# sourmash-bio/sourmash

Hardware: AMD Instinct MI355X
Metric: Gbase/s sketched (k=31, scaled=1000) (higher is better)
Workload: dtype u64; 1 GPU; C2: sketch synthetic random DNA resident in HBM as ASCII, per GPU 1000 records of 10000000 bases (10000000000 bases, 10000001000 bytes with their separators), k=31 scaled=1000 seed=42; one step = k-mer kernel + radix sort + unique; records_per_gpu=1000, record_len=10000000, bases_per_gpu=10000000000, bytes_per_gpu=10000001000, ksize=31, scaled=1000, unique_hashes_rank0=9998668, unique_hashes_job=9998668, collectives=none (the exchange runs with --full)

## Files before the change

sourmash_amd/csrc/capi_ingest.cpp:

```cpp
#include <stdio.h>
#include <algorithm>
#include <atomic>
#include <chrono>
#include "capi_common.hpp"
#include "ingest.hpp"
#include "pargz.hpp"
#include "residues.hpp"
#include "sigload.hpp"
#include "uniform_sort_core.hpp"

using namespace smg;

namespace {

static size_t sketch_ws_raw_bytes(uint64_t cap) { return al256(cap * 8); }
static size_t sketch_ws_sort_bytes(uint64_t cap, bool counts) {
    return std::max(sort_unique_temp_bytes(cap), sort_unique_uniform_temp_bound(cap, counts));
}

struct SortCounters { std::atomic<uint64_t> bucket{0}, small{0}, fellback{0}; };
static SortCounters& sort_counters() { static SortCounters c; return c; }

static void uniform_sort_and_report(const uint64_t* d_keys, const unsigned long long* d_n, uint64_t n_max, uint64_t thr, uint64_t* d_out,
                                    uint64_t* d_counts, uint64_t* d_n_out, void* d_head, void* d_tmp, size_t tmp_bytes, hipStream_t st,
                                    uint64_t report[3]) {
    uint64_t* d_report = (uint64_t*)d_head;
    uint32_t* d_flag = (uint32_t*)((char*)d_head + 64);
    hip_check(sort_unique_uniform(d_keys, d_n, n_max, thr, d_out, d_counts, d_n_out, d_flag, d_tmp, tmp_bytes, st), "sort_unique_uniform");
    hip_check(sort_report_launch(d_n, d_n_out, d_flag, d_report, st), "sort_report");
    hip_check(hipMemcpyAsync(report, d_report, 24, hipMemcpyDeviceToHost, st), "D2H");
    hip_check(hipStreamSynchronize(st), "sync");
}
static void count_sort_call(uint64_t n_max, uint64_t thr, size_t tmp_bytes, bool counts, bool fellback) {
    if (fellback) ++sort_counters().fellback;
    else if (sort_unique_uniform_form(n_max, thr, tmp_bytes, counts) == US_SMALL) ++sort_counters().small;
    else ++sort_counters().bucket;
}
static int key_bits(uint64_t thr) {
    int bits = 64;
    if (thr != ~0ull) { bits = 1; while (bits < 64 && (thr >> bits)) ++bits; }
    return bits;
}

}

extern "C" {

uint64_t smgpu_signature_add_file(SourmashSignature* p, const char* path, uint64_t* n_records) {
    return landing<uint64_t>([&]() -> uint64_t {
        if (!path) throw err_internal("null path");
        std::vector<KmerMinHash*> mhs;
        for (auto& mh : SIG(p)->sketches) mhs.push_back(&mh);
        uint64_t recs = 0, bases = 0;
        sketch_file_into(mhs, path, &recs, &bases);
        if (n_records) *n_records = recs;
        return bases;
    });
}
SourmashSignature** smgpu_sketch_files(const char* const* paths, uintptr_t n, const SourmashComputeParameters* params,
                                       uint32_t n_threads, uint64_t* total_bases) {
    return landing<SourmashSignature**>([&]() -> SourmashSignature** {
        if (!paths && n) throw err_internal("null paths");
        if (!CP(params)->dna || CP(params)->protein || CP(params)->dayhoff || CP(params)->hp)
// ... 77 lines not shown
        if (!path) throw err_internal("null path");
        std::vector<KmerMinHash*> mhs{MH(p)};
        uint64_t recs = 0, bases = 0;
        sketch_file_into(mhs, path, &recs, &bases);
        if (n_records) *n_records = recs;
        return bases;
    });
}

uint64_t smgpu_sketch_workspace_bytes(uint64_t out_capacity) {
    return (uint64_t)sketch_ws_raw_bytes(out_capacity) + 256 + sketch_ws_sort_bytes(out_capacity, false) + 512;
}

void smgpu_sort_counters(uint64_t* out) {
    if (!out) return;
    out[0] = sort_counters().bucket.load();
    out[1] = sort_counters().small.load();
    out[2] = sort_counters().fellback.load();
}

uint64_t smgpu_sketch_dna_raw(const uint8_t* d_seq, uint64_t len, uint32_t ksize, uint64_t seed, uint64_t max_hash,
                              uint64_t* d_out, uint64_t cap, uint64_t* d_result, void* d_ws, uint64_t ws_bytes,
                              void* stream) {
    uint64_t ret = ~0ull;
    landing_void([&] {
        hipStream_t st = (hipStream_t)stream;
        if (ws_bytes < smgpu_sketch_workspace_bytes(cap)) throw err_internal("workspace too small (smgpu_sketch_workspace_bytes)");
        uint64_t* d_raw = (uint64_t*)d_ws;
        void* d_head = (char*)d_ws + sketch_ws_raw_bytes(cap);
        void* d_tmp = (char*)d_head + 256;
        const size_t tmp_bytes = (size_t)(ws_bytes - sketch_ws_raw_bytes(cap) - 256);
        const uint64_t thr = max_hash ? max_hash : ~0ull;
        check_dna_ksize(ksize);
        hip_check(hipMemsetAsync(d_result, 0, 16, st), "memset");
        hip_check(sketch_dna_launch(d_seq, len, ksize, seed, thr, d_raw, (unsigned long long*)d_result, cap, st), "sketch_dna");
        uint64_t report[3] = {0, 0, 0};
        uniform_sort_and_report(d_raw, (const unsigned long long*)d_result, cap, thr, d_out, nullptr, d_result + 1, d_head, d_tmp, tmp_bytes,
                                st, report);
        const uint64_t kept = report[0];
        if (kept > cap)
            throw err_internal("output capacity too small: " + std::to_string(kept) + " kept hashes > capacity " + std::to_string(cap));
        count_sort_call(cap, thr, tmp_bytes, false, report[2] != 0);
        if (report[2] == 0) { ret = report[1]; return; }
        hip_check(sort_unique(d_raw, kept, d_out, nullptr, d_result + 1, d_tmp, tmp_bytes, key_bits(thr), st), "sort_unique");
        unsigned long long nu = 0;
        hip_check(hipMemcpyAsync(&nu, d_result + 1, 8, hipMemcpyDeviceToHost, st), "D2H");
        hip_check(hipStreamSynchronize(st), "sync");
        ret = nu;
    });
    return ret;
}

uint64_t smgpu_sort_unique_uniform_workspace_bytes(uint64_t n_max, int32_t counts) {
    return 256 + (uint64_t)sketch_ws_sort_bytes(n_max, counts != 0) + 512;
}

uint64_t smgpu_sort_unique_uniform_raw(uint64_t* d_keys, const uint64_t* d_n, uint64_t n_max, uint64_t thr, uint64_t* d_out, uint64_t* d_counts,
                                       uint64_t* d_result, void* d_ws, uint64_t ws_bytes, void* stream) {
    uint64_t ret = ~0ull;
    landing_void([&] {
        hipStream_t st = (hipStream_t)stream;
        if (!d_keys || !d_n || !d_out || !d_result || !d_ws) throw err_internal("null pointer");
        if (ws_bytes < smgpu_sort_unique_uniform_workspace_bytes(n_max, d_counts != nullptr))
            throw err_internal("workspace too small (smgpu_sort_unique_uniform_workspace_bytes)");
        void* d_tmp = (char*)d_ws + 256;
        const size_t tmp_bytes = (size_t)(ws_bytes - 256);
        uint64_t report[3] = {0, 0, 0};
        uniform_sort_and_report(d_keys, (const unsigned long long*)d_n, n_max, thr, d_out, d_counts, d_result, d_ws, d_tmp, tmp_bytes, st, report);
        count_sort_call(n_max, thr, tmp_bytes, d_counts != nullptr, report[2] != 0);
        if (report[2] == 0) { ret = report[1]; return; }
        const uint64_t n = std::min(report[0], n_max);
        hip_check(sort_unique(d_keys, n, d_out, d_counts, d_result, d_tmp, tmp_bytes, 64, st), "sort_unique");
        unsigned long long nu = 0;
        hip_check(hipMemcpyAsync(&nu, d_result, 8, hipMemcpyDeviceToHost, st), "D2H");
        hip_check(hipStreamSynchronize(st), "sync");
        ret = nu;
    });
    return ret;
}

uint64_t smgpu_sort_unique_raw(uint64_t* d_keys, uint64_t n, uint64_t* d_out, uint64_t* d_n_out, void* d_ws, uint64_t ws_bytes, void* stream) {
    uint64_t ret = ~0ull;
    landing_void([&] {
        hipStream_t st = (hipStream_t)stream;
        if (ws_bytes < sort_unique_temp_bytes(n)) throw err_internal("workspace too small (smgpu_sketch_workspace_bytes)");
        hip_check(sort_unique(d_keys, n, d_out, nullptr, d_n_out, d_ws, (size_t)ws_bytes, 64, st), "sort_unique");
        unsigned long long nu = 0;
        hip_check(hipMemcpyAsync(&nu, d_n_out, 8, hipMemcpyDeviceToHost, st), "D2H");
        hip_check(hipStreamSynchronize(st), "sync");
        ret = nu;
    });
    return ret;
}

void smgpu_sketch_dna_kernel_raw(const uint8_t* d_seq, uint64_t len, uint32_t ksize, uint64_t seed, uint64_t max_hash,
                                 uint64_t* d_out, uint64_t cap, uint64_t* d_count, void* stream) {
    landing_void([&] {
        check_dna_ksize(ksize);
        hip_check(sketch_dna_launch(d_seq, len, ksize, seed, max_hash ? max_hash : ~0ull, d_out,
                                    (unsigned long long*)d_count, cap, (hipStream_t)stream), "sketch_dna");
// ... 94 lines not shown
```

sourmash_amd/csrc/device_api.hpp:

```cpp
#pragma once
#include <hip/hip_runtime.h>
#include <stdint.h>
#include <stddef.h>
#include "find_core.hpp"
#include "qindex_core.hpp"

namespace smg {

inline size_t al256(size_t x) { return (x + 255) / 256 * 256; }
inline unsigned grid_for(uint64_t n, unsigned per, unsigned cap) {
    const uint64_t b = (n + per - 1) / per;
    return (unsigned)(b < 1 ? 1 : (b > cap ? cap : b));
}

hipError_t sketch_dna_launch(const uint8_t* d_seq, uint64_t len, uint32_t k, uint64_t seed, uint64_t thr,
                             uint64_t* d_out, unsigned long long* d_count, uint64_t cap, hipStream_t stream);
hipError_t sketch_dna_launch_grid(const uint8_t* d_seq, uint64_t len, uint32_t k, uint64_t seed, uint64_t thr,
                                  uint64_t* d_out, unsigned long long* d_count, uint64_t cap, uint32_t grid, hipStream_t stream);
struct SketchMultiOut { uint64_t thr; uint64_t* out; unsigned long long* count; uint64_t cap; };
bool sketch_dna_multi_supported(const uint32_t* ks, int n);
hipError_t sketch_dna_multi_launch(const uint8_t* d_new, uint64_t n_new, const uint32_t* ks, int n, uint64_t seed, const SketchMultiOut* outs,
                                   hipStream_t stream);
hipError_t sketch_dna_words_launch(const uint8_t* d_seq, uint64_t len, uint32_t k, uint64_t seed, uint64_t thr, uint64_t* d_out,
                                   unsigned long long* d_count, uint64_t cap, bool dense, hipStream_t stream);
// ... 2 lines not shown
                              uint64_t n_kmers, hipStream_t stream);
hipError_t first_invalid_launch(const uint8_t* d_seq, uint64_t len, unsigned long long* d_first, hipStream_t stream);

hipError_t hll_dna_launch(const uint8_t* d_seq, uint64_t len, uint32_t k, uint32_t p, uint32_t* d_regs, hipStream_t stream);
hipError_t hll_hashes_launch(const uint64_t* d_hashes, uint64_t n, uint32_t p, uint32_t* d_regs, bool skip_zero, hipStream_t stream);
hipError_t hll_pack_launch(const uint32_t* d_regs, uint32_t n, uint8_t* d_out, hipStream_t stream);

struct NgTable { uint64_t size, magic, off; };
struct NgDev {
    const NgTable* tabs = nullptr;
    uint32_t n_tables = 0;
    uint32_t* words = nullptr;
    uint64_t n_words = 0;
    uint64_t t0_words = 0;
    unsigned long long* occ = nullptr;
};
hipError_t nodegraph_dna_launch(const uint8_t* d_seq, uint64_t len, uint32_t k, const NgDev& g, hipStream_t stream);
hipError_t nodegraph_hashes_launch(const uint64_t* d_hashes, uint64_t n, const NgDev& g, hipStream_t stream);
hipError_t nodegraph_matches_launch(const uint64_t* d_hashes, const uint64_t* d_offsets, uint64_t n_rows, const NgDev& g,
                                    uint64_t* d_out, hipStream_t stream);

hipError_t residues_launch(const uint8_t* d_seq, uint64_t len, uint32_t hash_function, uint8_t* d_aa, hipStream_t stream);
uint64_t translated_bytes(uint64_t len);
hipError_t translate_launch(const uint8_t* d_seq, uint64_t len, uint32_t hash_function, uint8_t* d_aa, hipStream_t stream);
hipError_t residue_windows_launch(const uint8_t* d_aa, uint64_t n, uint32_t k, uint64_t seed, uint64_t thr, uint64_t* d_out,
                                  unsigned long long* d_count, uint64_t cap, bool dense, hipStream_t stream);

size_t sort_unique_temp_bytes(uint64_t n);
struct TagSegment { uint64_t src, dst, n; };
hipError_t tag_gather_launch(const uint64_t* d_src, const TagSegment* d_segs, uint32_t n_segs, uint64_t* d_dst, int hbits, hipStream_t stream);
hipError_t sort_unique(uint64_t* d_keys, uint64_t n, uint64_t* d_out, uint64_t* d_counts, uint64_t* d_n_out,
                       void* d_temp, size_t temp_bytes, int bits, hipStream_t stream);

hipError_t sort_unique_uniform(const uint64_t* d_keys, const unsigned long long* d_n, uint64_t n_max, uint64_t thr, uint64_t* d_out,
                               uint64_t* d_counts, uint64_t* d_n_out, uint32_t* d_fellback, void* d_temp, size_t temp_bytes,
                               hipStream_t stream);
size_t sort_unique_uniform_temp_bytes(uint64_t n_max, uint64_t thr, bool counts);
size_t sort_unique_uniform_temp_bound(uint64_t n_max, bool counts);
uint32_t sort_unique_uniform_form(uint64_t n_max, uint64_t thr, size_t temp_bytes, bool counts);
hipError_t sort_report_launch(const unsigned long long* d_n, const uint64_t* d_n_out, const uint32_t* d_fellback, uint64_t* d_report,
                              hipStream_t stream);

size_t sort_pairs_temp_bytes(uint64_t n);
hipError_t sort_pairs(const uint64_t* d_keys_in, uint64_t* d_keys_out, const uint64_t* d_vals_in, uint64_t* d_vals_out, uint64_t n,
                      int bits, void* d_temp, size_t temp_bytes, hipStream_t stream);
size_t rle_pairs_temp_bytes(uint64_t n);
hipError_t rle_pairs(const uint64_t* d_a, const uint64_t* d_b, uint64_t n, uint64_t* d_out_a, uint64_t* d_out_b, uint64_t* d_counts,
                     uint64_t* d_n_out, void* d_temp, size_t temp_bytes, hipStream_t stream);

hipError_t records_pairs_launch(const uint8_t* d_seq, uint64_t len, uint32_t k, uint64_t seed, uint64_t thr, uint64_t* d_hash,
                                uint64_t* d_pos, unsigned long long* d_count, uint64_t cap, hipStream_t stream);
hipError_t records_check_starts_launch(const uint64_t* d_starts, uint64_t n_records, uint64_t len, unsigned long long* d_bad,
                                       hipStream_t stream);
size_t records_csr_temp_bytes(uint64_t n_pairs);
hipError_t records_csr_launch(uint64_t* d_pair_hash, uint64_t* d_pair_pos, uint64_t n_pairs, const uint64_t* d_starts, uint64_t n_records,
                              uint32_t k, uint64_t max_hash, uint64_t* d_hashes, uint64_t* d_abunds, uint64_t* d_offsets, uint64_t* d_n_out,
                              void* d_temp, size_t temp_bytes, hipStream_t stream);

hipError_t records_csr_ends_launch(uint64_t* d_pair_hash, uint64_t* d_pair_pos, uint64_t n_pairs, const uint64_t* d_starts, const uint64_t* d_ends,
                                   uint64_t n_records, uint32_t k, uint64_t max_hash, uint64_t* d_hashes, uint64_t* d_abunds, uint64_t* d_offsets,
                                   uint64_t* d_n_out, void* d_temp, size_t temp_bytes, hipStream_t stream);
hipError_t records_check_ends_launch(const uint64_t* d_starts, const uint64_t* d_ends, uint64_t n_records, unsigned long long* d_bad,
                                     hipStream_t stream);
hipError_t records_file_ends_launch(const uint64_t* d_starts, uint64_t n_records, uint64_t* d_ends, hipStream_t stream);

hipError_t residue_pairs_launch(const uint8_t* d_aa, uint64_t n_bound, const uint64_t* d_n, uint32_t k, uint64_t seed, uint64_t thr,
                                uint64_t* d_hash, uint64_t* d_pos, unsigned long long* d_count, uint64_t cap, hipStream_t stream);
uint64_t translated_records_bytes_bound(uint64_t len, uint64_t n_records);
size_t translate_records_temp_bytes(uint64_t n_records);
hipError_t translate_records_launch(const uint8_t* d_seq, uint64_t len, const uint64_t* d_starts, const uint64_t* d_ends, uint64_t n_records,
                                    uint32_t hash_function, uint64_t* d_block_starts, uint8_t* d_aa, void* d_temp, size_t temp_bytes,
                                    hipStream_t stream);

hipError_t find_dir_launch(const uint64_t* d_q, uint64_t n, uint32_t shift, uint64_t n_buckets, uint32_t* d_dir, hipStream_t stream);
// ... 153 lines not shown
```

sourmash_amd/csrc/uniform_sort.hip:

```cpp
#include <hip/hip_runtime.h>
#include "device_api.hpp"
#include "uniform_sort_core.hpp"

namespace smg {
namespace {

constexpr uint32_t NO_BASE = 0xffffffffu;

__device__ __forceinline__ uint64_t us_count(const unsigned long long* d_n, uint64_t n_max) {
    const uint64_t n = *d_n;
    return n < n_max ? n : n_max;
}

template <int T>
__device__ __forceinline__ void us_sort_lds(uint64_t* keys, uint32_t n) {
    const uint32_t P = us_pow2(n);
    for (uint32_t k = 2, j = 0; k <= P; us_next_step(k, j)) {
        for (uint32_t t = threadIdx.x; t < P / 2; t += T) {
            uint32_t a, b;
            us_pair(t, k, j, a, b);
            us_compare_exchange(keys, n, a, b);
        }
        __syncthreads();
    }
}

template <int T>
__device__ __forceinline__ uint32_t us_block_scan(uint32_t v, uint32_t* wsum, uint32_t& total) {
    const uint32_t lane = threadIdx.x & 63, wave = threadIdx.x >> 6;
    uint32_t x = v;
#pragma unroll
    for (uint32_t off = 1; off < 64; off <<= 1) {
        const uint32_t y = __shfl_up(x, off);
        if (lane >= off) x += y;
    }
    if (lane == 63) wsum[wave] = x;
    __syncthreads();
    uint32_t base = 0, all = 0;
#pragma unroll
    for (uint32_t w = 0; w < T / 64; ++w) {
        const uint32_t t = wsum[w];
        if (w < wave) base += t;
        all += t;
    }
    __syncthreads();
    total = all;
    return base + x - v;
}

template <int T, int E, int B, bool LEAF>
__device__ __forceinline__ void us_sort_keys(const uint64_t* src, uint32_t n, uint32_t bin_shift, uint64_t* s, uint32_t* bins,
                                             uint32_t* wsum) {
    constexpr int BPT = B / T;
    static_assert(B % T == 0, "bins per thread");
#pragma unroll
    for (int i = 0; i < BPT; ++i) bins[threadIdx.x + i * T] = 0;
    __syncthreads();
    uint64_t key[E];
    uint32_t at[E];
#pragma unroll
    for (int e = 0; e < E; ++e) {
        const uint32_t i = threadIdx.x + e * T;
        key[e] = 0;
        at[e] = 0;
        if (i < n) {
            key[e] = src[i];
            at[e] = atomicAdd(&bins[LEAF ? us_bin_leaf(bin_shift, key[e]) : us_bin_small(bin_shift, key[e])], 1u);
        }
    }
    __syncthreads();
    uint32_t mine[BPT], sum = 0, most = 0;
#pragma unroll
    for (int i = 0; i < BPT; ++i) {
        mine[i] = bins[threadIdx.x * BPT + i];
        sum += mine[i];
        most = mine[i] > most ? mine[i] : most;
    }
    uint32_t total;
    uint32_t start = us_block_scan<T>(sum, wsum, total);
    if (__syncthreads_or(most > US_BIN_LIMIT)) {
#pragma unroll
        for (int e = 0; e < E; ++e)
            if (threadIdx.x + e * T < n) s[threadIdx.x + e * T] = key[e];
        __syncthreads();
        us_sort_lds<T>(s, n);
        return;
    }
#pragma unroll
    for (int i = 0; i < BPT; ++i) {
        bins[threadIdx.x * BPT + i] = start;
        start += mine[i];
    }
    if (threadIdx.x == T - 1) bins[B] = start;
    __syncthreads();
#pragma unroll
    for (int e = 0; e < E; ++e) {
        if (threadIdx.x + e * T >= n) continue;
        at[e] += bins[LEAF ? us_bin_leaf(bin_shift, key[e]) : us_bin_small(bin_shift, key[e])];
        s[at[e]] = key[e];
// ... 18 lines not shown
template <int T, int E, typename CT>
__device__ __forceinline__ uint32_t us_unique_write(const uint64_t* keys, uint32_t n, uint32_t* scan, uint64_t* out, CT* counts) {
    const uint32_t lo = threadIdx.x * E;
    uint32_t heads = 0;
#pragma unroll
    for (int e = 0; e < E; ++e)
        if (lo + e < n && us_is_head(keys, lo + e)) ++heads;
    uint32_t total;
    const uint32_t first = us_block_scan<T>(heads, scan, total);
    uint32_t q = first;
#pragma unroll
    for (int e = 0; e < E; ++e) {
        const uint32_t i = lo + e;
        if (i < n && us_is_head(keys, i)) {
            out[q] = keys[i];
            if (counts) counts[q] = (CT)0 - (CT)i;
            ++q;
        }
    }
    if (counts) {
        __syncthreads();
        q = first;
#pragma unroll
        for (int e = 0; e < E; ++e) {
            const uint32_t i = lo + e;
            if (i >= n) break;
            if (us_is_head(keys, i)) ++q;
            if (us_is_tail(keys, n, i)) counts[q - 1] += (CT)(i + 1);
        }
    }
    return total;
}

__global__ __launch_bounds__(1024) void us_small_kernel(const uint64_t* __restrict__ keys, const unsigned long long* __restrict__ d_n,
                                                        uint64_t n_max, uint32_t small_shift, uint64_t* __restrict__ out,
                                                        uint64_t* __restrict__ counts, uint64_t* __restrict__ d_n_out,
                                                        uint32_t* __restrict__ d_fellback) {
    __shared__ uint64_t s[US_SMALL_MAX];
    __shared__ uint32_t bins[US_SMALL_BINS + 1];
    __shared__ uint32_t scan[1024 / 64];
    const uint32_t n = (uint32_t)us_count(d_n, n_max < US_SMALL_MAX ? n_max : US_SMALL_MAX);
    us_sort_keys<1024, US_SMALL_MAX / 1024, US_SMALL_BINS, false>(keys, n, small_shift, s, bins, scan);
    const uint32_t total = us_unique_write<1024, US_SMALL_MAX / 1024, uint64_t>(s, n, scan, out, counts);
    if (threadIdx.x == 0) {
        *d_n_out = total;
        *d_fellback = 0;
    }
}

template <bool SECOND>
__global__ __launch_bounds__(256) void us_scatter_kernel(const UsPlan p, const uint64_t* __restrict__ src,
                                                         const unsigned long long* __restrict__ d_n, uint64_t n_max,
                                                         const uint32_t* __restrict__ src_cursor, uint32_t tiles_per_region,
                                                         uint32_t* __restrict__ cursor, uint64_t* __restrict__ dst, uint64_t dst_cap,
                                                         uint32_t* __restrict__ d_fellback) {
    __shared__ uint32_t hist[US_FANOUT];
    __shared__ uint32_t base[US_FANOUT];
    uint64_t region = 0, begin, n;
    if (!SECOND) {
        n = us_count(d_n, n_max);
        begin = (uint64_t)blockIdx.x * US_TILE;
    } else {
        __shared__ uint32_t quit;
        if (threadIdx.x == 0) quit = *d_fellback;
        __syncthreads();
        if (quit) return;
        region = blockIdx.x / tiles_per_region;
        const uint64_t held = src_cursor[region];
        n = held < p.region_cap ? held : p.region_cap;
        begin = (uint64_t)(blockIdx.x % tiles_per_region) * US_TILE;
        src += region * p.region_cap;
        cursor += region * US_FANOUT;
        dst += region * US_FANOUT * dst_cap;
    }
    if (begin >= n) return;
    hist[threadIdx.x] = 0;
    __syncthreads();
    constexpr int E = US_TILE / 256;
    uint64_t key[E];
    uint32_t digit[E], rank[E];
    bool stray = false;
#pragma unroll
    for (int e = 0; e < E; ++e) {
        const uint64_t i = begin + (uint64_t)e * 256 + threadIdx.x;
        digit[e] = US_FANOUT;
        rank[e] = 0;
        key[e] = 0;
        if (i < n) {
            key[e] = src[i];
            digit[e] = SECOND ? us_digit_second(p, region, key[e]) : us_digit_first(p, key[e]);
            if (digit[e] < US_FANOUT) rank[e] = atomicAdd(&hist[digit[e]], 1u);
            else stray = true;
        }
    }
    if (stray) atomicOr(d_fellback, 1u);
    __syncthreads();
    {
        const uint32_t c = hist[threadIdx.x];
        uint32_t b = NO_BASE;
        if (c) {
            const uint32_t at = atomicAdd(&cursor[threadIdx.x], c);
            if (us_reserve_ok(at, c, dst_cap)) b = at;
            else atomicOr(d_fellback, 1u);
        }
        base[threadIdx.x] = b;
    }
    __syncthreads();
#pragma unroll
    for (int e = 0; e < E; ++e) {
        if (digit[e] >= US_FANOUT) continue;
        const uint32_t b = base[digit[e]];
        if (b != NO_BASE) dst[(uint64_t)digit[e] * dst_cap + b + rank[e]] = key[e];
    }
}

__global__ __launch_bounds__(256) void us_leaf_kernel(uint32_t shift, const uint32_t* __restrict__ cursor, uint64_t* __restrict__ leaves,
                                                      uint32_t* __restrict__ leaf_counts, uint32_t* __restrict__ leaf_distinct,
                                                      const uint32_t* __restrict__ d_fellback) {
    __shared__ uint64_t s[US_LEAF_CAP];
    __shared__ uint32_t bins[US_LEAF_BINS + 1];
    __shared__ uint32_t scan[256 / 64];
    if (*d_fellback) return;
    const uint64_t leaf = blockIdx.x;
    const uint32_t held = cursor[leaf];
    const uint32_t n = held < US_LEAF_CAP ? held : US_LEAF_CAP;
    uint64_t* mine = leaves + leaf * US_LEAF_CAP;
    us_sort_keys<256, US_LEAF_CAP / 256, US_LEAF_BINS, true>(mine, n, shift, s, bins, scan);
    const uint32_t total = us_unique_write<256, US_LEAF_CAP / 256, uint32_t>(s, n, scan, mine,
                                                                            leaf_counts ? leaf_counts + leaf * US_LEAF_CAP : nullptr);
    if (threadIdx.x == 0) leaf_distinct[leaf] = total;
}

__global__ __launch_bounds__(1024) void us_scan_kernel(const uint32_t* __restrict__ leaf_distinct, uint32_t n_leaves,
                                                       uint32_t* __restrict__ offsets, uint64_t* __restrict__ d_n_out,
                                                       const uint32_t* __restrict__ d_fellback) {
    __shared__ uint32_t wsum[1024 / 64];
    if (*d_fellback) return;
    uint32_t carry = 0;
    for (uint32_t base = 0; base < n_leaves; base += 4096) {
        const uint32_t l = base + threadIdx.x * 4;
        uint32_t v[4], sum = 0, total;
#pragma unroll
        for (int i = 0; i < 4; ++i) {
            v[i] = l + i < n_leaves ? leaf_distinct[l + i] : 0;
            sum += v[i];
        }
        uint32_t at = carry + us_block_scan<1024>(sum, wsum, total);
#pragma unroll
        for (int i = 0; i < 4; ++i) {
            if (l + i < n_leaves) offsets[l + i] = at;
            at += v[i];
        }
        carry += total;
    }
    if (threadIdx.x == 0) {
        offsets[n_leaves] = carry;
        *d_n_out = carry;
    }
}

__global__ __launch_bounds__(256) void us_pack_kernel(const uint64_t* __restrict__ leaves, const uint32_t* __restrict__ leaf_counts,
                                                      const uint32_t* __restrict__ offsets, uint64_t* __restrict__ out,
                                                      uint64_t* __restrict__ counts, const uint32_t* __restrict__ d_fellback) {
    if (*d_fellback) return;
    const uint64_t leaf = blockIdx.x;
    const uint32_t at = offsets[leaf], n = offsets[leaf + 1] - at;
    for (uint32_t i = threadIdx.x; i < n; i += 256) {
        out[at + i] = leaves[leaf * US_LEAF_CAP + i];
        if (counts) counts[at + i] = leaf_counts[leaf * US_LEAF_CAP + i];
    }
}

__global__ void us_report_kernel(const unsigned long long* __restrict__ d_n, const uint64_t* __restrict__ d_n_out,
                                 const uint32_t* __restrict__ d_fellback, uint64_t* __restrict__ report) {
    report[0] = *d_n;
    report[1] = *d_n_out;
    report[2] = *d_fellback;
}

size_t up256(size_t x) { return (x + 255) / 256 * 256; }

struct UsLayout {
    size_t coarse_cursors, leaf_cursors, cursor_bytes, distinct, offsets, coarse, leaves, counts, total;
};
UsLayout us_layout(const UsPlan& p, bool counts) {
    UsLayout y{};
    const size_t n_leaf_cursors = p.form == US_TWO_PASS ? (size_t)p.regions * US_FANOUT : US_FANOUT;
    y.coarse_cursors = 0;
    y.leaf_cursors = up256(US_FANOUT * 4);
    y.cursor_bytes = y.leaf_cursors + up256(n_leaf_cursors * 4);
    y.distinct = y.cursor_bytes;
    y.offsets = y.distinct + up256(n_leaf_cursors * 4);
    y.coarse = y.offsets + up256((n_leaf_cursors + 1) * 4);
    y.leaves = y.coarse + up256((size_t)p.regions * p.region_cap * 8);
    y.counts = y.leaves + up256((size_t)p.leaves * US_LEAF_CAP * 8);
    y.total = y.counts + (counts ? up256((size_t)p.leaves * US_LEAF_CAP * 4) : 0);
    return y;
}

}

size_t sort_unique_uniform_temp_bytes(uint64_t n_max, uint64_t thr, bool counts) {
    const UsPlan p = us_plan(n_max, thr);
    if (p.form == US_SMALL || p.form == US_DECLINE) return 256;
    return us_layout(p, counts).total;
}

size_t sort_unique_uniform_temp_bound(uint64_t n_max, bool counts) {
    if (n_max <= US_SMALL_MAX) return 256;
    return up256((size_t)n_max * 8 * 5 + (counts ? (size_t)n_max * 4 * 3 : 0) + ((size_t)8 << 20));
}

uint32_t sort_unique_uniform_form(uint64_t n_max, uint64_t thr, size_t temp_bytes, bool counts) {
    const UsPlan p = us_plan(n_max, thr);
    if (p.form == US_SMALL || p.form == US_DECLINE) return p.form;
    return temp_bytes < us_layout(p, counts).total ? (uint32_t)US_DECLINE : p.form;
}

hipError_t sort_unique_uniform(const uint64_t* d_keys, const unsigned long long* d_n, uint64_t n_max, uint64_t thr, uint64_t* d_out,
                               uint64_t* d_counts, uint64_t* d_n_out, uint32_t* d_fellback, void* d_temp, size_t temp_bytes,
                               hipStream_t stream) {
    const UsPlan p = us_plan(n_max, thr);
    const uint32_t form = sort_unique_uniform_form(n_max, thr, temp_bytes, d_counts != nullptr);
    if (form == US_SMALL) {
        hipLaunchKernelGGL(us_small_kernel, dim3(1), dim3(1024), 0, stream, d_keys, d_n, n_max, us_small_shift(thr), d_out, d_counts, d_n_out,
                           d_fellback);
        return hipGetLastError();
    }
    if (form == US_DECLINE) return hipMemsetD32Async((hipDeviceptr_t)d_fellback, 1, 1, stream);
    const UsLayout y = us_layout(p, d_counts != nullptr);
    char* base = (char*)d_temp;
    uint32_t* coarse_cursors = (uint32_t*)(base + y.coarse_cursors);
    uint32_t* leaf_cursors = (uint32_t*)(base + y.leaf_cursors);
    uint32_t* distinct = (uint32_t*)(base + y.distinct);
    uint32_t* offsets = (uint32_t*)(base + y.offsets);
    uint64_t* coarse = (uint64_t*)(base + y.coarse);
    uint64_t* leaves = (uint64_t*)(base + y.leaves);
    uint32_t* leaf_counts = d_counts ? (uint32_t*)(base + y.counts) : nullptr;
    hipError_t e = hipMemsetAsync(d_fellback, 0, 4, stream);
    if (e != hipSuccess) return e;
    e = hipMemsetAsync(base, 0, y.cursor_bytes, stream);
    if (e != hipSuccess) return e;
    const uint32_t tiles = (uint32_t)((n_max + US_TILE - 1) / US_TILE);
    if (form == US_ONE_PASS) {
        hipLaunchKernelGGL(us_scatter_kernel<false>, dim3(tiles), dim3(256), 0, stream, p, d_keys, d_n, n_max, (const uint32_t*)nullptr, 1u,
                           leaf_cursors, leaves, (uint64_t)US_LEAF_CAP, d_fellback);
    } else {
        hipLaunchKernelGGL(us_scatter_kernel<false>, dim3(tiles), dim3(256), 0, stream, p, d_keys, d_n, n_max, (const uint32_t*)nullptr, 1u,
                           coarse_cursors, coarse, p.region_cap, d_fellback);
        const uint32_t tpr = (uint32_t)((p.region_cap + US_TILE - 1) / US_TILE);
        hipLaunchKernelGGL(us_scatter_kernel<true>, dim3((uint32_t)p.regions * tpr), dim3(256), 0, stream, p, (const uint64_t*)coarse, d_n,
                           n_max, (const uint32_t*)coarse_cursors, tpr, leaf_cursors, leaves, (uint64_t)US_LEAF_CAP, d_fellback);
    }
    const uint32_t L = (uint32_t)p.leaves;
    hipLaunchKernelGGL(us_leaf_kernel, dim3(L), dim3(256), 0, stream, p.shift, (const uint32_t*)leaf_cursors, leaves, leaf_counts, distinct,
                       (const uint32_t*)d_fellback);
    hipLaunchKernelGGL(us_scan_kernel, dim3(1), dim3(1024), 0, stream, (const uint32_t*)distinct, L, offsets, d_n_out,
                       (const uint32_t*)d_fellback);
    hipLaunchKernelGGL(us_pack_kernel, dim3(L), dim3(256), 0, stream, (const uint64_t*)leaves, (const uint32_t*)leaf_counts,
                       (const uint32_t*)offsets, d_out, d_counts, (const uint32_t*)d_fellback);
    return hipGetLastError();
}

hipError_t sort_report_launch(const unsigned long long* d_n, const uint64_t* d_n_out, const uint32_t* d_fellback, uint64_t* d_report,
                              hipStream_t stream) {
    hipLaunchKernelGGL(us_report_kernel, dim3(1), dim3(1), 0, stream, d_n, d_n_out, d_fellback, d_report);
    return hipGetLastError();
}

}
```

sourmash_amd/csrc/uniform_sort_core.hpp:

```cpp
#pragma once
#include <stdint.h>

#if defined(__HIPCC__)
#include <hip/hip_runtime.h>
#endif

#ifndef SMG_HD
#if defined(__HIPCC__)
#define SMG_HD __host__ __device__ __forceinline__
#else
#define SMG_HD inline
#endif
#endif

namespace smg {

constexpr uint32_t US_SMALL_MAX = 16384;
constexpr uint32_t US_LEAF_CAP = 1024;
constexpr uint32_t US_FANOUT = 256;
constexpr uint32_t US_TILE = 4096;
constexpr uint64_t US_MAX_LEAVES = (uint64_t)US_FANOUT * US_FANOUT;

enum UsForm : uint32_t { US_DECLINE = 0, US_SMALL = 1, US_ONE_PASS = 2, US_TWO_PASS = 3 };

// ... 24 lines not shown
    UsPlan p{US_DECLINE, 0, 0, 0, 0, thr};
    if (n_max <= US_SMALL_MAX) { p.form = US_SMALL; return p; }
    if (n_max > 0xffffffffull) return p;
    int shift = 63;
    for (; shift >= 0; --shift) {
        const uint64_t L = us_leaves(thr, (uint32_t)shift);
        if (L > US_MAX_LEAVES) return p;
        if (us_load_fits((n_max + L - 1) / L, US_LEAF_CAP)) break;
    }
    if (shift < 0) return p;
    p.shift = (uint32_t)shift;
    p.leaves = us_leaves(thr, p.shift);
    if (p.leaves <= US_FANOUT) { p.form = US_ONE_PASS; return p; }
    p.form = US_TWO_PASS;
    p.regions = ((p.leaves - 1) >> 8) + 1;
    const uint64_t load = ((n_max + p.leaves - 1) / p.leaves) * US_FANOUT;
    p.region_cap = load + 8 * us_isqrt_up(load);
    return p;
}

SMG_HD uint64_t us_leaf_of(const UsPlan& p, uint64_t key) { return key >> p.shift; }
SMG_HD uint32_t us_digit_first(const UsPlan& p, uint64_t key) {
    if (key > p.thr) return US_FANOUT;
    const uint64_t leaf = us_leaf_of(p, key);
    return (uint32_t)(p.form == US_TWO_PASS ? leaf >> 8 : leaf);
}
SMG_HD uint32_t us_digit_second(const UsPlan& p, uint64_t region, uint64_t key) {
    if (key > p.thr) return US_FANOUT;
    const uint64_t leaf = us_leaf_of(p, key);
    return (leaf >> 8) == region ? (uint32_t)(leaf & 0xff) : US_FANOUT;
}
SMG_HD bool us_reserve_ok(uint64_t base, uint64_t count, uint64_t cap) { return base <= cap && count <= cap - base; }

constexpr uint32_t US_LEAF_BINS = 1024;
constexpr uint32_t US_SMALL_BINS = 4096;
constexpr uint32_t US_BIN_LIMIT = 32;
SMG_HD uint32_t us_bin_leaf(uint32_t shift, uint64_t key) { return (uint32_t)(key >> (shift > 10 ? shift - 10 : 0)) & (US_LEAF_BINS - 1); }
SMG_HD uint32_t us_small_shift(uint64_t thr) {
    uint32_t s = 0;
    while (s < 63 && (thr >> s) >= US_SMALL_BINS) ++s;
    return s;
}
SMG_HD uint32_t us_bin_small(uint32_t small_shift, uint64_t key) {
    const uint64_t b = key >> small_shift;
    return b < US_SMALL_BINS ? (uint32_t)b : US_SMALL_BINS - 1;
}
SMG_HD bool us_before(uint64_t other, uint32_t other_at, uint64_t key, uint32_t at) { return other < key || (other == key && other_at < at); }

SMG_HD uint32_t us_pow2(uint32_t n) {
    uint32_t p = 1;
    while (p < n) p <<= 1;
    return p;
}
SMG_HD void us_pair(uint32_t t, uint32_t k, uint32_t j, uint32_t& a, uint32_t& b) {
    const uint32_t off = t & ((j == 0 ? k >> 1 : j) - 1);
    a = 2 * (t - off) + off;
    b = j == 0 ? 2 * (t - off) + k - 1 - off : a + j;
}
SMG_HD void us_compare_exchange(uint64_t* keys, uint32_t n, uint32_t a, uint32_t b) {
    if (b >= n) return;
    const uint64_t x = keys[a], y = keys[b];
    if (x > y) { keys[a] = y; keys[b] = x; }
}
SMG_HD void us_next_step(uint32_t& k, uint32_t& j) {
    if (j == 0) j = k >> 2; else j >>= 1;
    if (j == 0) k <<= 1;
// ... 7 lines not shown
```

Before: 384.9 Gbase/s.

## Restructure uniform sort scatter into persistent staged kernel and fold report writes

```diff
diff --git a/sourmash_amd/csrc/capi_ingest.cpp b/sourmash_amd/csrc/capi_ingest.cpp
--- a/sourmash_amd/csrc/capi_ingest.cpp
+++ b/sourmash_amd/csrc/capi_ingest.cpp
@@ -24,11 +24,8 @@
 static void uniform_sort_and_report(const uint64_t* d_keys, const unsigned long long* d_n, uint64_t n_max, uint64_t thr, uint64_t* d_out,
                                     uint64_t* d_counts, uint64_t* d_n_out, void* d_head, void* d_tmp, size_t tmp_bytes, hipStream_t st,
                                     uint64_t report[3]) {
-    uint64_t* d_report = (uint64_t*)d_head;
-    uint32_t* d_flag = (uint32_t*)((char*)d_head + 64);
-    hip_check(sort_unique_uniform(d_keys, d_n, n_max, thr, d_out, d_counts, d_n_out, d_flag, d_tmp, tmp_bytes, st), "sort_unique_uniform");
-    hip_check(sort_report_launch(d_n, d_n_out, d_flag, d_report, st), "sort_report");
-    hip_check(hipMemcpyAsync(report, d_report, 24, hipMemcpyDeviceToHost, st), "D2H");
+    hip_check(sort_unique_uniform(d_keys, d_n, n_max, thr, d_out, d_counts, d_n_out, d_head, d_tmp, tmp_bytes, st), "sort_unique_uniform");
+    hip_check(hipMemcpyAsync(report, (const char*)d_head + US_HEAD_REPORT, 24, hipMemcpyDeviceToHost, st), "D2H");
     hip_check(hipStreamSynchronize(st), "sync");
 }
 static void count_sort_call(uint64_t n_max, uint64_t thr, size_t tmp_bytes, bool counts, bool fellback) {
@@ -172,7 +169,7 @@
         const size_t tmp_bytes = (size_t)(ws_bytes - sketch_ws_raw_bytes(cap) - 256);
         const uint64_t thr = max_hash ? max_hash : ~0ull;
         check_dna_ksize(ksize);
-        hip_check(hipMemsetAsync(d_result, 0, 16, st), "memset");
+        hip_check(sort_unique_uniform_prepare(cap, thr, false, d_head, d_tmp, tmp_bytes, d_result, st), "sort_unique_uniform_prepare");
         hip_check(sketch_dna_launch(d_seq, len, ksize, seed, thr, d_raw, (unsigned long long*)d_result, cap, st), "sketch_dna");
         uint64_t report[3] = {0, 0, 0};
         uniform_sort_and_report(d_raw, (const unsigned long long*)d_result, cap, thr, d_out, nullptr, d_result + 1, d_head, d_tmp, tmp_bytes,
@@ -206,6 +203,7 @@
         void* d_tmp = (char*)d_ws + 256;
         const size_t tmp_bytes = (size_t)(ws_bytes - 256);
         uint64_t report[3] = {0, 0, 0};
+        hip_check(sort_unique_uniform_prepare(n_max, thr, d_counts != nullptr, d_ws, d_tmp, tmp_bytes, nullptr, st), "sort_unique_uniform_prepare");
         uniform_sort_and_report(d_keys, (const unsigned long long*)d_n, n_max, thr, d_out, d_counts, d_result, d_ws, d_tmp, tmp_bytes, st, report);
         count_sort_call(n_max, thr, tmp_bytes, d_counts != nullptr, report[2] != 0);
         if (report[2] == 0) { ret = report[1]; return; }
diff --git a/sourmash_amd/csrc/device_api.hpp b/sourmash_amd/csrc/device_api.hpp
--- a/sourmash_amd/csrc/device_api.hpp
+++ b/sourmash_amd/csrc/device_api.hpp
@@ -58,14 +58,15 @@
 hipError_t sort_unique(uint64_t* d_keys, uint64_t n, uint64_t* d_out, uint64_t* d_counts, uint64_t* d_n_out,
                        void* d_temp, size_t temp_bytes, int bits, hipStream_t stream);
 
+constexpr size_t US_HEAD_REPORT = 0;
+constexpr size_t US_HEAD_FLAG = 64;
+hipError_t sort_unique_uniform_prepare(uint64_t n_max, uint64_t thr, bool counts, void* d_head, void* d_temp, size_t temp_bytes,
+                                       uint64_t* d_result, hipStream_t stream);
 hipError_t sort_unique_uniform(const uint64_t* d_keys, const unsigned long long* d_n, uint64_t n_max, uint64_t thr, uint64_t* d_out,
-                               uint64_t* d_counts, uint64_t* d_n_out, uint32_t* d_fellback, void* d_temp, size_t temp_bytes,
-                               hipStream_t stream);
+                               uint64_t* d_counts, uint64_t* d_n_out, void* d_head, void* d_temp, size_t temp_bytes, hipStream_t stream);
 size_t sort_unique_uniform_temp_bytes(uint64_t n_max, uint64_t thr, bool counts);
 size_t sort_unique_uniform_temp_bound(uint64_t n_max, bool counts);
 uint32_t sort_unique_uniform_form(uint64_t n_max, uint64_t thr, size_t temp_bytes, bool counts);
-hipError_t sort_report_launch(const unsigned long long* d_n, const uint64_t* d_n_out, const uint32_t* d_fellback, uint64_t* d_report,
-                              hipStream_t stream);
 
 size_t sort_pairs_temp_bytes(uint64_t n);
 hipError_t sort_pairs(const uint64_t* d_keys_in, uint64_t* d_keys_out, const uint64_t* d_vals_in, uint64_t* d_vals_out, uint64_t n,
diff --git a/sourmash_amd/csrc/uniform_sort.hip b/sourmash_amd/csrc/uniform_sort.hip
--- a/sourmash_amd/csrc/uniform_sort.hip
+++ b/sourmash_amd/csrc/uniform_sort.hip
@@ -1,4 +1,5 @@
 #include <hip/hip_runtime.h>
+#include <stdlib.h>
 #include "device_api.hpp"
 #include "uniform_sort_core.hpp"
 
@@ -48,9 +49,18 @@
     return base + x - v;
 }
 
-template <int T, int E, int B, bool LEAF>
-__device__ __forceinline__ void us_sort_keys(const uint64_t* src, uint32_t n, uint32_t bin_shift, uint64_t* s, uint32_t* bins,
-                                             uint32_t* wsum) {
+template <int T, int E>
+__device__ __forceinline__ void us_load_keys(const uint64_t* src, uint32_t n, uint64_t (&key)[E]) {
+#pragma unroll
+    for (int e = 0; e < E; ++e) {
+        const uint32_t i = threadIdx.x + e * T;
+        key[e] = i < n ? src[i] : 0;
+    }
+}
+
+template <int T, int E, int B, bool LEAF, bool LOAD>
+__device__ __forceinline__ void us_sort_keys(const uint64_t (&held)[E], const uint64_t* src, uint32_t n, uint32_t bin_shift, uint64_t* s,
+                                             uint32_t* bins, uint32_t* wsum) {
     constexpr int BPT = B / T;
     static_assert(B % T == 0, "bins per thread");
 #pragma unroll
@@ -61,10 +71,10 @@
 #pragma unroll
     for (int e = 0; e < E; ++e) {
         const uint32_t i = threadIdx.x + e * T;
-        key[e] = 0;
         at[e] = 0;
+        key[e] = LOAD ? 0 : held[e];
         if (i < n) {
-            key[e] = src[i];
+            if (LOAD) key[e] = src[i];
             at[e] = atomicAdd(&bins[LEAF ? us_bin_leaf(bin_shift, key[e]) : us_bin_small(bin_shift, key[e])], 1u);
         }
     }
@@ -149,91 +159,188 @@
     return total;
 }
 
+__device__ __forceinline__ void us_write_report(void* d_head, uint64_t count, uint64_t distinct, uint32_t fellback) {
+    uint64_t* report = (uint64_t*)((char*)d_head + US_HEAD_REPORT);
+    report[0] = count;
+    report[1] = distinct;
+    report[2] = fellback;
+}
+__device__ __forceinline__ uint32_t* us_head_flag(void* d_head) { return (uint32_t*)((char*)d_head + US_HEAD_FLAG); }
+
+__global__ __launch_bounds__(256) void us_zero_kernel(uint32_t* __restrict__ words, uint32_t n_words, void* __restrict__ d_head,
+                                                      uint32_t* __restrict__ d_result32) {
+    const uint32_t i = blockIdx.x * 256 + threadIdx.x;
+    if (i < n_words) words[i] = 0;
+    if (i == 0) *us_head_flag(d_head) = 0;
+    if (d_result32 && i >= 1 && i < 5) d_result32[i - 1] = 0;
+}
+
+__global__ void us_decline_kernel(const unsigned long long* __restrict__ d_n, void* __restrict__ d_head) {
+    *us_head_flag(d_head) = 1;
+    us_write_report(d_head, *d_n, 0, 1);
+}
+
 __global__ __launch_bounds__(1024) void us_small_kernel(const uint64_t* __restrict__ keys, const unsigned long long* __restrict__ d_n,
                                                         uint64_t n_max, uint32_t small_shift, uint64_t* __restrict__ out,
                                                         uint64_t* __restrict__ counts, uint64_t* __restrict__ d_n_out,
-                                                        uint32_t* __restrict__ d_fellback) {
+                                                        void* __restrict__ d_head) {
     __shared__ uint64_t s[US_SMALL_MAX];
     __shared__ uint32_t bins[US_SMALL_BINS + 1];
     __shared__ uint32_t scan[1024 / 64];
     const uint32_t n = (uint32_t)us_count(d_n, n_max < US_SMALL_MAX ? n_max : US_SMALL_MAX);
-    us_sort_keys<1024, US_SMALL_MAX / 1024, US_SMALL_BINS, false>(keys, n, small_shift, s, bins, scan);
+    const uint64_t none[US_SMALL_MAX / 1024] = {};
+    us_sort_keys<1024, US_SMALL_MAX / 1024, US_SMALL_BINS, false, true>(none, keys, n, small_shift, s, bins, scan);
     const uint32_t total = us_unique_write<1024, US_SMALL_MAX / 1024, uint64_t>(s, n, scan, out, counts);
     if (threadIdx.x == 0) {
         *d_n_out = total;
-        *d_fellback = 0;
-    }
-}
+        *us_head_flag(d_head) = 0;
+        us_write_report(d_head, *d_n, total, 0);
+    }
+}
+
+struct UsTileAt {
+    const uint64_t* src;
+    uint32_t n;
+    uint32_t region;
+};
 
 template <bool SECOND>
-__global__ __launch_bounds__(256) void us_scatter_kernel(const UsPlan p, const uint64_t* __restrict__ src,
+__global__ __launch_bounds__(256, 4) void us_scatter_kernel(const UsPlan p, const uint64_t* __restrict__ src,
                                                          const unsigned long long* __restrict__ d_n, uint64_t n_max,
-                                                         const uint32_t* __restrict__ src_cursor, uint32_t tiles_per_region,
-                                                         uint32_t* __restrict__ cursor, uint64_t* __restrict__ dst, uint64_t dst_cap,
-                                                         uint32_t* __restrict__ d_fellback) {
-    __shared__ uint32_t hist[US_FANOUT];
-    __shared__ uint32_t base[US_FANOUT];
-    uint64_t region = 0, begin, n;
-    if (!SECOND) {
-        n = us_count(d_n, n_max);
-        begin = (uint64_t)blockIdx.x * US_TILE;
-    } else {
-        __shared__ uint32_t quit;
+                                                         const uint32_t* __restrict__ src_cursor, uint32_t* __restrict__ cursor,
+                                                         uint64_t* __restrict__ dst, uint64_t dst_cap, uint32_t* __restrict__ d_fellback) {
+    constexpr int E = US_TILE / 256;
+    __shared__ uint64_t stage[US_TILE];
+    __shared__ uint32_t hist[US_FANOUT * US_HIST_STRIDE];
+    __shared__ uint32_t lstart[US_FANOUT + 1];
+    __shared__ uint32_t tile_start[SECOND ? US_FANOUT + 1 : 1];
+    __shared__ uint32_t wsum[256 / 64];
+    __shared__ uint32_t quit;
+    const uint64_t n_first = us_count(d_n, n_max);
+    uint64_t n_tiles = us_tiles(n_first);
+    if (SECOND) {
+        if (blockIdx.x >= n_tiles + p.regions) return;
+        uint32_t mine = 0;
+        if (threadIdx.x < p.regions) {
+            const uint64_t held = src_cursor[threadIdx.x];
+            mine = (uint32_t)us_tiles(held < p.region_cap ? held : p.region_cap);
+        }
         if (threadIdx.x == 0) quit = *d_fellback;
+        uint32_t all;
+        const uint32_t at = us_block_scan<256>(mine, wsum, all);
+        tile_start[threadIdx.x] = at;
+        if (threadIdx.x == 255) tile_start[US_FANOUT] = all;
         __syncthreads();
         if (quit) return;
-        region = blockIdx.x / tiles_per_region;
-        const uint64_t held = src_cursor[region];
-        n = held < p.region_cap ? held : p.region_cap;
-        begin = (uint64_t)(blockIdx.x % tiles_per_region) * US_TILE;
-        src += region * p.region_cap;
-        cursor += region * US_FANOUT;
-        dst += region * US_FANOUT * dst_cap;
-    }
-    if (begin >= n) return;
-    hist[threadIdx.x] = 0;
-    __syncthreads();
-    constexpr int E = US_TILE / 256;
-    uint64_t key[E];
-    uint32_t digit[E], rank[E];
-    bool stray = false;
-#pragma unroll
-    for (int e = 0; e < E; ++e) {
-        const uint64_t i = begin + (uint64_t)e * 256 + threadIdx.x;
-        digit[e] = US_FANOUT;
-        rank[e] = 0;
-        key[e] = 0;
-        if (i < n) {
-            key[e] = src[i];
-            digit[e] = SECOND ? us_digit_second(p, region, key[e]) : us_digit_first(p, key[e]);
-            if (digit[e] < US_FANOUT) rank[e] = atomicAdd(&hist[digit[e]], 1u);
-            else stray = true;
-        }
-    }
-    if (stray) atomicOr(d_fellback, 1u);
-    __syncthreads();
-    {
-        const uint32_t c = hist[threadIdx.x];
-        uint32_t b = NO_BASE;
-        if (c) {
-            const uint32_t at = atomicAdd(&cursor[threadIdx.x], c);
-            if (us_reserve_ok(at, c, dst_cap)) b = at;
-            else atomicOr(d_fellback, 1u);
-        }
-        base[threadIdx.x] = b;
-    }
-    __syncthreads();
-#pragma unroll
-    for (int e = 0; e < E; ++e) {
-        if (digit[e] >= US_FANOUT) continue;
-        const uint32_t b = base[digit[e]];
-        if (b != NO_BASE) dst[(uint64_t)digit[e] * dst_cap + b + rank[e]] = key[e];
+        n_tiles = all;
+    }
+    if (blockIdx.x >= n_tiles) return;
+
+    auto tile_at = [&](uint64_t t) {
+        UsTileAt a;
+        if constexpr (!SECOND) {
+            const uint64_t begin = t * US_TILE, left = n_first - begin;
+            a.src = src + begin;
+            a.n = (uint32_t)(left < US_TILE ? left : US_TILE);
+            a.region = 0;
+        } else {
+            a.region = us_tile_region(tile_start, (uint32_t)t);
+            const uint64_t held = src_cursor[a.region];
+            const uint64_t n = held < p.region_cap ? held : p.region_cap;
+            const uint64_t begin = (t - tile_start[a.region]) * US_TILE, left = n - begin;
+            a.src = src + a.region * p.region_cap + begin;
+            a.n = (uint32_t)(left < US_TILE ? left : US_TILE);
+        }
+        return a;
+    };
+    auto load = [&](const UsTileAt& a, uint64_t (&key)[E]) {
+#pragma unroll
+        for (int e = 0; e < E; ++e) {
+            const uint32_t i = (uint32_t)e * 256 + threadIdx.x;
+            key[e] = i < a.n ? a.src[i] : 0;
+        }
+    };
+
+    const uint32_t sub = us_sub(threadIdx.x);
+#pragma unroll
+    for (uint32_t s = 0; s < US_SUBS; ++s) hist[us_hist_at(threadIdx.x, s)] = 0;
+    uint64_t key[E], next_key[E];
+    UsTileAt cur = tile_at(blockIdx.x), next = cur;
+    load(cur, key);
+    __syncthreads();
+    for (uint64_t t = blockIdx.x; t < n_tiles; t += gridDim.x) {
+        const bool more = t + gridDim.x < n_tiles;
+        if (threadIdx.x == 0) quit = __hip_atomic_load(d_fellback, __ATOMIC_RELAXED, __HIP_MEMORY_SCOPE_AGENT);
+        if (more) {
+            next = tile_at(t + gridDim.x);
+            load(next, next_key);
+        }
+        uint32_t* my_cursor = cursor + (SECOND ? (uint64_t)cur.region * US_FANOUT : 0);
+        uint64_t* my_dst = dst + (SECOND ? (uint64_t)cur.region * US_FANOUT * dst_cap : 0);
+        uint32_t where[E];
+        bool stray = false;
+#pragma unroll
+        for (int e = 0; e < E; ++e) {
+            where[e] = US_FANOUT << 12;
+            if ((uint32_t)e * 256 + threadIdx.x < cur.n) {
+                const uint32_t digit = SECOND ? us_digit_second(p, cur.region, key[e]) : us_digit_first(p, key[e]);
+                if (digit < US_FANOUT) where[e] = digit << 12 | atomicAdd(&hist[us_hist_at(digit, sub)], 1u);
+                else stray = true;
+            }
+        }
+        if (stray) atomicOr(d_fellback, 1u);
+        __syncthreads();
+        if (quit) return;
+        uint32_t c = 0;
+#pragma unroll
+        for (uint32_t s = 0; s < US_SUBS; ++s) {
+            const uint32_t v = hist[us_hist_at(threadIdx.x, s)];
+            hist[us_hist_at(threadIdx.x, s)] = c;
+            c += v;
+        }
+        {
+            uint32_t b = NO_BASE;
+            if (c) {
+                const uint32_t at = atomicAdd(&my_cursor[threadIdx.x], c);
+                if (us_reserve_ok(at, c, dst_cap)) b = at;
+                else atomicOr(d_fellback, 1u);
+            }
+            hist[us_hist_at(threadIdx.x, US_SUBS)] = b;
+        }
+        uint32_t placed;
+        const uint32_t first = us_block_scan<256>(c, wsum, placed);
+        lstart[threadIdx.x] = first;
+        __syncthreads();
+#pragma unroll
+        for (int e = 0; e < E; ++e) {
+            const uint32_t digit = where[e] >> 12;
+            if (digit < US_FANOUT) stage[lstart[digit] + hist[us_hist_at(digit, sub)] + (where[e] & 0xfffu)] = key[e];
+        }
+        __syncthreads();
+#pragma unroll
+        for (uint32_t s = 0; s < US_SUBS; ++s) hist[us_hist_at(threadIdx.x, s)] = 0;
+#pragma unroll
+        for (int e = 0; e < E; ++e) {
+            const uint32_t j = (uint32_t)e * 256 + threadIdx.x;
+            if (j >= placed) continue;
+            const uint64_t k = stage[j];
+            const uint32_t digit = SECOND ? us_digit_second(p, cur.region, k) : us_digit_first(p, k);
+            const uint32_t b = hist[us_hist_at(digit, US_SUBS)];
+            if (b != NO_BASE) my_dst[(uint64_t)digit * dst_cap + b + (j - lstart[digit])] = k;
+        }
+        if (more) {
+#pragma unroll
+            for (int e = 0; e < E; ++e) key[e] = next_key[e];
+            cur = next;
+        }
+        __syncthreads();
     }
 }
 
 __global__ __launch_bounds__(256) void us_leaf_kernel(uint32_t shift, const uint32_t* __restrict__ cursor, uint64_t* __restrict__ leaves,
                                                       uint32_t* __restrict__ leaf_counts, uint32_t* __restrict__ leaf_distinct,
                                                       const uint32_t* __restrict__ d_fellback) {
+    constexpr int E = US_LEAF_CAP / 256;
     __shared__ uint64_t s[US_LEAF_CAP];
     __shared__ uint32_t bins[US_LEAF_BINS + 1];
     __shared__ uint32_t scan[256 / 64];
@@ -242,29 +349,33 @@
     const uint32_t held = cursor[leaf];
     const uint32_t n = held < US_LEAF_CAP ? held : US_LEAF_CAP;
     uint64_t* mine = leaves + leaf * US_LEAF_CAP;
-    us_sort_keys<256, US_LEAF_CAP / 256, US_LEAF_BINS, true>(mine, n, shift, s, bins, scan);
-    const uint32_t total = us_unique_write<256, US_LEAF_CAP / 256, uint32_t>(s, n, scan, mine,
-                                                                            leaf_counts ? leaf_counts + leaf * US_LEAF_CAP : nullptr);
+    uint64_t key[E];
+    us_load_keys<256, E>(mine, n, key);
+    us_sort_keys<256, E, US_LEAF_BINS, true, false>(key, nullptr, n, shift, s, bins, scan);
+    const uint32_t total = us_unique_write<256, E, uint32_t>(s, n, scan, mine, leaf_counts ? leaf_counts + leaf * US_LEAF_CAP : nullptr);
     if (threadIdx.x == 0) leaf_distinct[leaf] = total;
 }
 
 __global__ __launch_bounds__(1024) void us_scan_kernel(const uint32_t* __restrict__ leaf_distinct, uint32_t n_leaves,
-                                                       uint32_t* __restrict__ offsets, uint64_t* __restrict__ d_n_out,
-                                                       const uint32_t* __restrict__ d_fellback) {
+                                                       uint32_t* __restrict__ offsets, const unsigned long long* __restrict__ d_n,
+                                                       uint64_t* __restrict__ d_n_out, void* __restrict__ d_head) {
     __shared__ uint32_t wsum[1024 / 64];
-    if (*d_fellback) return;
+    if (*us_head_flag(d_head)) {
+        if (threadIdx.x == 0) us_write_report(d_head, *d_n, 0, 1);
+        return;
+    }
     uint32_t carry = 0;
-    for (uint32_t base = 0; base < n_leaves; base += 4096) {
-        const uint32_t l = base + threadIdx.x * 4;
-        uint32_t v[4], sum = 0, total;
-#pragma unroll
-        for (int i = 0; i < 4; ++i) {
+    for (uint32_t base = 0; base < n_leaves; base += 1024 * US_SCAN_PER_LANE) {
+        const uint32_t l = base + threadIdx.x * US_SCAN_PER_LANE;
+        uint32_t v[US_SCAN_PER_LANE], sum = 0, total;
+#pragma unroll
+        for (uint32_t i = 0; i < US_SCAN_PER_LANE; ++i) {
             v[i] = l + i < n_leaves ? leaf_distinct[l + i] : 0;
             sum += v[i];
         }
         uint32_t at = carry + us_block_scan<1024>(sum, wsum, total);
 #pragma unroll
-        for (int i = 0; i < 4; ++i) {
+        for (uint32_t i = 0; i < US_SCAN_PER_LANE; ++i) {
             if (l + i < n_leaves) offsets[l + i] = at;
             at += v[i];
         }
@@ -273,6 +384,7 @@
     if (threadIdx.x == 0) {
         offsets[n_leaves] = carry;
         *d_n_out = carry;
+        us_write_report(d_head, *d_n, carry, 0);
     }
 }
 
@@ -286,13 +398,6 @@
         out[at + i] = leaves[leaf * US_LEAF_CAP + i];
         if (counts) counts[at + i] = leaf_counts[leaf * US_LEAF_CAP + i];
     }
-}
-
-__global__ void us_report_kernel(const unsigned long long* __restrict__ d_n, const uint64_t* __restrict__ d_n_out,
-                                 const uint32_t* __restrict__ d_fellback, uint64_t* __restrict__ report) {
-    report[0] = *d_n;
-    report[1] = *d_n_out;
-    report[2] = *d_fellback;
 }
 
 size_t up256(size_t x) { return (x + 255) / 256 * 256; }
@@ -334,17 +439,61 @@
     return temp_bytes < us_layout(p, counts).total ? (uint32_t)US_DECLINE : p.form;
 }
 
+namespace {
+
+unsigned us_grid_cap() {
+    static const unsigned cap = [] {
+        const char* e = getenv("SMG_US_GRID");
+        const long v = e ? atol(e) : 0;
+        return v > 0 ? (unsigned)v : 0xffffffffu;
+    }();
+    return cap;
+}
+
+unsigned us_resident(const void* kernel) {
+    int per_cu = 0, dev = 0, cus = 0;
+    if (hipOccupancyMaxActiveBlocksPerMultiprocessor(&per_cu, kernel, 256, 0) != hipSuccess || hipGetDevice(&dev) != hipSuccess ||
+        hipDeviceGetAttribute(&cus, hipDeviceAttributeMultiprocessorCount, dev) != hipSuccess || per_cu < 1 || cus < 1) {
+        (void)hipGetLastError();
+        return 1024u;
+    }
+    return (unsigned)per_cu * (unsigned)cus;
+}
+unsigned us_grid(unsigned resident, uint64_t work) {
+    uint64_t g = resident < us_grid_cap() ? resident : us_grid_cap();
+    if (g > work) g = work;
+    return g ? (unsigned)g : 1u;
+}
+
+}
+
+hipError_t sort_unique_uniform_prepare(uint64_t n_max, uint64_t thr, bool counts, void* d_head, void* d_temp, size_t temp_bytes,
+                                       uint64_t* d_result, hipStream_t stream) {
+    const uint32_t form = sort_unique_uniform_form(n_max, thr, temp_bytes, counts);
+    uint32_t n_words = 0;
+    if (form == US_ONE_PASS || form == US_TWO_PASS) n_words = (uint32_t)(us_layout(us_plan(n_max, thr), counts).cursor_bytes / 4);
+    else if (!d_result) return hipSuccess;
+    const uint32_t blocks = n_words > 5 ? (n_words + 255) / 256 : 1;
+    hipLaunchKernelGGL(us_zero_kernel, dim3(blocks), dim3(256), 0, stream, (uint32_t*)d_temp, n_words, d_head, (uint32_t*)d_result);
+    return hipGetLastError();
+}
+
 hipError_t sort_unique_uniform(const uint64_t* d_keys, const unsigned long long* d_n, uint64_t n_max, uint64_t thr, uint64_t* d_out,
-                               uint64_t* d_counts, uint64_t* d_n_out, uint32_t* d_fellback, void* d_temp, size_t temp_bytes,
-                               hipStream_t stream) {
+                               uint64_t* d_counts, uint64_t* d_n_out, void* d_head, void* d_temp, size_t temp_bytes, hipStream_t stream) {
     const UsPlan p = us_plan(n_max, thr);
     const uint32_t form = sort_unique_uniform_form(n_max, thr, temp_bytes, d_counts != nullptr);
+    uint32_t* d_fellback = (uint32_t*)((char*)d_head + US_HEAD_FLAG);
     if (form == US_SMALL) {
         hipLaunchKernelGGL(us_small_kernel, dim3(1), dim3(1024), 0, stream, d_keys, d_n, n_max, us_small_shift(thr), d_out, d_counts, d_n_out,
-                           d_fellback);
+                           d_head);
         return hipGetLastError();
     }
-    if (form == US_DECLINE) return hipMemsetD32Async((hipDeviceptr_t)d_fellback, 1, 1, stream);
+    if (form == US_DECLINE) {
+        hipLaunchKernelGGL(us_decline_kernel, dim3(1), dim3(1), 0, stream, d_n, d_head);
+        return hipGetLastError();
+    }
+    static const unsigned resident_first = us_resident((const void*)us_scatter_kernel<false>);
+    static const unsigned resident_second = us_resident((const void*)us_scatter_kernel<true>);
     const UsLayout y = us_layout(p, d_counts != nullptr);
     char* base = (char*)d_temp;
     uint32_t* coarse_cursors = (uint32_t*)(base + y.coarse_cursors);
@@ -354,35 +503,24 @@
     uint64_t* coarse = (uint64_t*)(base + y.coarse);
     uint64_t* leaves = (uint64_t*)(base + y.leaves);
     uint32_t* leaf_counts = d_counts ? (uint32_t*)(base + y.counts) : nullptr;
-    hipError_t e = hipMemsetAsync(d_fellback, 0, 4, stream);
-    if (e != hipSuccess) return e;
-    e = hipMemsetAsync(base, 0, y.cursor_bytes, stream);
-    if (e != hipSuccess) return e;
-    const uint32_t tiles = (uint32_t)((n_max + US_TILE - 1) / US_TILE);
+    const uint64_t tiles = us_tiles(n_max);
     if (form == US_ONE_PASS) {
-        hipLaunchKernelGGL(us_scatter_kernel<false>, dim3(tiles), dim3(256), 0, stream, p, d_keys, d_n, n_max, (const uint32_t*)nullptr, 1u,
-                           leaf_cursors, leaves, (uint64_t)US_LEAF_CAP, d_fellback);
+        hipLaunchKernelGGL(us_scatter_kernel<false>, dim3(us_grid(resident_first, tiles)), dim3(256), 0, stream, p, d_keys, d_n, n_max,
+                           (const uint32_t*)nullptr, leaf_cursors, leaves, (uint64_t)US_LEAF_CAP, d_fellback);
     } else {
-        hipLaunchKernelGGL(us_scatter_kernel<false>, dim3(tiles), dim3(256), 0, stream, p, d_keys, d_n, n_max, (const uint32_t*)nullptr, 1u,
-                           coarse_cursors, coarse, p.region_cap, d_fellback);
-        const uint32_t tpr = (uint32_t)((p.region_cap + US_TILE - 1) / US_TILE);
-        hipLaunchKernelGGL(us_scatter_kernel<true>, dim3((uint32_t)p.regions * tpr), dim3(256), 0, stream, p, (const uint64_t*)coarse, d_n,
-                           n_max, (const uint32_t*)coarse_cursors, tpr, leaf_cursors, leaves, (uint64_t)US_LEAF_CAP, d_fellback);
+        hipLaunchKernelGGL(us_scatter_kernel<false>, dim3(us_grid(resident_first, tiles)), dim3(256), 0, stream, p, d_keys, d_n, n_max,
+                           (const uint32_t*)nullptr, coarse_cursors, coarse, p.region_cap, d_fellback);
+        hipLaunchKernelGGL(us_scatter_kernel<true>, dim3(us_grid(resident_second, tiles + p.regions)), dim3(256), 0, stream, p,
+                           (const uint64_t*)coarse, d_n, n_max, (const uint32_t*)coarse_cursors, leaf_cursors, leaves, (uint64_t)US_LEAF_CAP,
+                           d_fellback);
     }
     const uint32_t L = (uint32_t)p.leaves;
     hipLaunchKernelGGL(us_leaf_kernel, dim3(L), dim3(256), 0, stream, p.shift, (const uint32_t*)leaf_cursors, leaves, leaf_counts, distinct,
                        (const uint32_t*)d_fellback);
-    hipLaunchKernelGGL(us_scan_kernel, dim3(1), dim3(1024), 0, stream, (const uint32_t*)distinct, L, offsets, d_n_out,
-                       (const uint32_t*)d_fellback);
+    hipLaunchKernelGGL(us_scan_kernel, dim3(1), dim3(1024), 0, stream, (const uint32_t*)distinct, L, offsets, d_n, d_n_out, d_head);
     hipLaunchKernelGGL(us_pack_kernel, dim3(L), dim3(256), 0, stream, (const uint64_t*)leaves, (const uint32_t*)leaf_counts,
                        (const uint32_t*)offsets, d_out, d_counts, (const uint32_t*)d_fellback);
     return hipGetLastError();
 }
 
-hipError_t sort_report_launch(const unsigned long long* d_n, const uint64_t* d_n_out, const uint32_t* d_fellback, uint64_t* d_report,
-                              hipStream_t stream) {
-    hipLaunchKernelGGL(us_report_kernel, dim3(1), dim3(1), 0, stream, d_n, d_n_out, d_fellback, d_report);
-    return hipGetLastError();
-}
-
-}
+}
diff --git a/sourmash_amd/csrc/uniform_sort_core.hpp b/sourmash_amd/csrc/uniform_sort_core.hpp
--- a/sourmash_amd/csrc/uniform_sort_core.hpp
+++ b/sourmash_amd/csrc/uniform_sort_core.hpp
@@ -80,6 +80,22 @@
 }
 SMG_HD bool us_reserve_ok(uint64_t base, uint64_t count, uint64_t cap) { return base <= cap && count <= cap - base; }
 
+SMG_HD uint64_t us_tiles(uint64_t n) { return (n + US_TILE - 1) / US_TILE; }
+SMG_HD uint32_t us_tile_region(const uint32_t* tile_start, uint32_t t) {
+    uint32_t lo = 0, hi = US_FANOUT;
+    while (hi - lo > 1) {
+        const uint32_t mid = (lo + hi) >> 1;
+        if (tile_start[mid] <= t) lo = mid; else hi = mid;
+    }
+    return lo;
+}
+constexpr uint32_t US_SUBS = 4;
+constexpr uint32_t US_HIST_STRIDE = US_SUBS + 1;
+SMG_HD uint32_t us_sub(uint32_t lane) { return lane & (US_SUBS - 1); }
+SMG_HD uint32_t us_hist_at(uint32_t digit, uint32_t sub) { return digit * US_HIST_STRIDE + sub; }
+
+constexpr uint32_t US_SCAN_PER_LANE = 4;
+
 constexpr uint32_t US_LEAF_BINS = 1024;
 constexpr uint32_t US_SMALL_BINS = 4096;
 constexpr uint32_t US_BIN_LIMIT = 32;
```

After: 385.5 Gbase/s, median of 6. No clear change (+0.2%).
